# evandez/neuron-descriptions

Hardware: AMD Instinct MI355X
Metric: neuron-descriptions/sec (whole node), 4096 neurons x k=15 exemplars (higher is better)
Workload: dtype f32-equivalent: operands split into (hi,lo) f16 pairs (22 significant bits), 3 f16 MFMAs per product, f32 accumulate

## Files before the change

### neuron-descriptions_amd/csrc/chain.hip

```cpp
#include "common.h"

#include <cstdlib>

namespace milan {

typedef float f32x16 __attribute__((ext_vector_type(16)));
typedef float f32x4 __attribute__((ext_vector_type(4)));
typedef _Float16 f16x8 __attribute__((ext_vector_type(8)));

#define GLOBAL_AS __attribute__((address_space(1)))
#define LDS_AS __attribute__((address_space(3)))

namespace {

__device__ inline f16x8 h8(f32x4 v) { return __builtin_bit_cast(f16x8, v); }

__device__ inline void chain_split8(const float* v, f32x4* hi_out, f32x4* lo_out) {
  split8_rne(v, hi_out, lo_out);
}
__device__ inline void chain_join8(f32x4 hi, f32x4 lo, float* v) { join8_exact(hi, lo, v); }

constexpr int kSRow = 68;
constexpr int kTileFloats = 64 * 64;
constexpr int kConvMaxW = 56;
constexpr int kConvSlots = (256 + 2 * (kConvMaxW + 1) + 3) / 4 * 4;

template <int N>
__device__ __forceinline__ void wait_vmcnt() {
  asm volatile("s_waitcnt vmcnt(%0)" ::"n"(N) : "memory");
}

}

template <int P, int NW, bool RES_LDS, int KD, bool XACC, bool PROF = false, int NR = P,
          bool CONV = false, bool C1 = false>
__global__ __launch_bounds__(NW * 64, NW / 4) void chain_kernel(ChainArgs g) {
  long long tprof[8] = {0, 0, 0, 0, 0, 0, 0, 0};
  long long tlast = 0;
  auto stamp = [&](int k) {
    if constexpr (PROF) {
      const long long t = __builtin_readcyclecounter();
      tprof[k] += t - tlast;
      tlast = t;
    }
  };
  if constexpr (PROF) tlast = __builtin_readcyclecounter();
  constexpr int N3 = 4 * P, N1 = NR;
  constexpr int K3 = P + KD;
  constexpr int KS3 = K3 / 16;
  constexpr int NSLAB = N3 / 64;
  constexpr int T3 = K3 / 64;
  constexpr bool RES = KD == 0;
  static_assert(!(RES_LDS && !RES) && K3 % 64 == 0, "chain: configuration");
  constexpr int T1 = N1 / 64;
  constexpr int L = T3 + T1;
  constexpr int NT1 = N1 / 32;
  constexpr int STAGES = RES_LDS ? 7 : 4, AHEAD = STAGES - 1;
  constexpr int INFL = AHEAD - 2;
  constexpr int PIECES = 16 / NW;
  constexpr int C_OPS = RES_LDS ? 8 : (RES ? 10 : 2);
  static_assert(P % 64 == 0 && (NW == 4 || NW == 8), "chain: configuration");
  static_assert(!CONV || (P == 64 && NW == 8 && !RES_LDS), "chain: the conv front needs planes 64");
  static_assert(!C1 || CONV, "chain: c1 in front needs the conv front");
  constexpr int Q1 = C1 ? 1 : 0;
  constexpr int QC = CONV ? 9 + Q1 : 0;
  extern __shared__ __attribute__((aligned(16))) float smem[];

  const int tid = threadIdx.x;
  const int lane = tid & 63;
  const int wave = __builtin_amdgcn_readfirstlane(tid >> 6);
  const int px = lane & 31, half = lane >> 5;
  float sat = 0.f;
  float* ring = smem;
  float* strip = smem + STAGES * kTileFloats + wave * (32 * kSRow);
  float* rstrip = strip;
  float* biasl = smem + STAGES * kTileFloats + NW * (32 * kSRow);

  g.M = live_rows(g.m_live, g.m_live_mul, g.M);
  if ((long)blockIdx.x * (NW * 32) >= g.M) return;
  const long m0 = (long)blockIdx.x * (NW * 32) + wave * 32;
  const long mfrag = (m0 + px < g.M) ? m0 + px : (long)g.M - 1;
  const bool tail = (long)(blockIdx.x + 1) * (NW * 32) > g.M;

  const int lrow = lane >> 4;
  const int lpos = lane & 15;
  auto issue_tile = [&](int q) {
    constexpr int NTILES = QC + NSLAB * L;
    q = q < NTILES ? q : NTILES - 1;
    const float* base;
    long ld;
    if (C1 && q == 0) {
      base = g.W0; ld = 64;
    } else if (CONV && q < QC) {
      base = g.W2 + 64 * (q - Q1); ld = 9 * 64;
    } else {
      const int qc = q - QC;
      const int j = qc / L, qq = qc - j * L;
      if (qq < T3) { base = g.W3 + (long)(64 * j) * K3 + 64 * qq; ld = K3; }
      else { base = g.W1 + (long)(64 * (qq - T3)) * N3 + 64 * j; ld = N3; }
    }
    float* slot = ring + (q % STAGES) * kTileFloats;
#pragma unroll
    for (int i = 0; i < PIECES; ++i) {
      const int pc = wave * PIECES + i;
      const int rr = 4 * pc + lrow;
      const int c = lpos ^ (rr & 15);
      __builtin_amdgcn_global_load_lds(
          (const GLOBAL_AS void*)(base + (long)rr * ld + c * 4),
          (LDS_AS void*)(slot + pc * 256), 16, 0, 0);
    }
  };

  f32x4 t2h[KS3], t2l[KS3];
  float* const cin = smem + STAGES * kTileFloats;
  float* const czero = cin + kConvSlots * 64;
  f32x4 bias2v[CONV ? 8 : 1], bias0v[C1 ? 8 : 1];
  if constexpr (C1) {
#pragma unroll
    for (int s4 = 0; s4 < 4; ++s4) {
      bias0v[2 * s4] = *reinterpret_cast<const f32x4*>(g.bias0 + 16 * s4 + 8 * half);
      bias0v[2 * s4 + 1] = *reinterpret_cast<const f32x4*>(g.bias0 + 16 * s4 + 8 * half + 4);
    }
  }
  if constexpr (CONV) {
    const long wg0 = (long)blockIdx.x * (NW * 32);
    const int nslots = NW * 32 + 2 * (g.cw + 1);
    const int npieces = (nslots + 3) >> 2;
    for (int pc = wave; pc < npieces; pc += NW) {
      const int sl = 4 * pc + lrow;
      long m = wg0 - (g.cw + 1) + sl;
      m = m < 0 ? 0 : (m < g.M ? m : (long)g.M - 1);
      const int c = lpos ^ (sl & 15);
      __builtin_amdgcn_global_load_lds((const GLOBAL_AS void*)(g.C2in + m * 64 + c * 4),
                                       (LDS_AS void*)(cin + pc * 256), 16, 0, 0);
    }
    if (tid < 16) *reinterpret_cast<f32x4*>(czero + tid * 4) = f32x4{0.f, 0.f, 0.f, 0.f};
#pragma unroll
    for (int s4 = 0; s4 < 4; ++s4) {
      bias2v[2 * s4] = *reinterpret_cast<const f32x4*>(g.bias2 + 16 * s4 + 8 * half);
      bias2v[2 * s4 + 1] = *reinterpret_cast<const f32x4*>(g.bias2 + 16 * s4 + 8 * half + 4);
    }
  }
  {
    if constexpr (!CONV) {
    const float* tp = g.T2 + mfrag * P + half * 8;
#pragma unroll
    for (int s = 0; s < P / 16; ++s) {
      t2h[s] = *reinterpret_cast<const f32x4*>(tp + s * 16);
      t2l[s] = *reinterpret_cast<const f32x4*>(tp + s * 16 + 4);
    }
    }
    if constexpr (KD > 0) {
      const float* ap = g.A2 + mfrag * KD + half * 8;
#pragma unroll
      for (int s = 0; s < KD / 16; ++s) {
        t2h[P / 16 + s] = *reinterpret_cast<const f32x4*>(ap + s * 16);
        t2l[P / 16 + s] = *reinterpret_cast<const f32x4*>(ap + s * 16 + 4);
      }
    }
  }
  const int erow = lane >> 3, ecol = (lane & 7) * 8;
  f32x4 res[RES_LDS ? 1 : 4][2], bias3v[2];
  auto load_res = [&](int j) {
    if constexpr (!RES_LDS) {
      const int n = 64 * j + ecol;
      bias3v[0] = *reinterpret_cast<const f32x4*>(g.bias3 + n);
      bias3v[1] = *reinterpret_cast<const f32x4*>(g.bias3 + n + 4);
      if constexpr (!RES) return;
#pragma unroll
      for (int it = 0; it < 4; ++it) {
        long m = m0 + it * 8 + erow;
        m = m < g.M ? m : (long)g.M - 1;
        const float* rp = g.R + m * N3 + n;
        res[it][0] = *reinterpret_cast<const f32x4*>(rp);
        res[it][1] = *reinterpret_cast<const f32x4*>(rp + 4);
      }
      return;
    }
#pragma unroll
    for (int i = 0; i < 8; ++i) {
      const int r = 4 * i + lrow;
      long m = m0 + r;
      m = m < g.M ? m : (long)g.M - 1;
      const int c = lpos ^ (r & 1);
      __builtin_amdgcn_global_load_lds(
          (const GLOBAL_AS void*)(g.R + m * N3 + 64 * j + c * 4),
          (LDS_AS void*)(rstrip + i * 256), 16, 0, 0);
    }
  };
  if constexpr (RES_LDS) {
    for (int i = tid; i < N3; i += NW * 64) biasl[i] = g.bias3[i];
  }
  load_res(0);
#pragma unroll
  for (int t = 0; t < AHEAD; ++t) issue_tile(t);

  f32x16 acc1[NT1], acc1x[XACC ? NT1 : 1];
#pragma unroll
  for (int u = 0; u < NT1; ++u)
#pragma unroll
    for (int r = 0; r < 16; ++r) {
      acc1[u][r] = 0.f;
      if constexpr (XACC) acc1x[u][r] = 0.f;
    }

  const int fsw = px & 15;
  auto wfrag = [&](const float* slot, int t, int c) -> f32x4 {
    return *reinterpret_cast<const f32x4*>(slot + (32 * t + px) * 64 + ((c ^ fsw) << 2));
  };

  auto to_strip = [&](const f32x16& a, int t) {
#pragma unroll
    for (int qd = 0; qd < 4; ++qd) {
      f32x4 v = {a[4 * qd], a[4 * qd + 1], a[4 * qd + 2], a[4 * qd + 3]};
      *reinterpret_cast<f32x4*>(strip + px * kSRow + 32 * t + 8 * qd + 4 * half) = v;
    }
  };

  wait_vmcnt<INFL * PIECES>();
  asm volatile("s_waitcnt lgkmcnt(0)" ::: "memory");
  __builtin_amdgcn_s_barrier();
  stamp(0);
#pragma unroll
  for (int s = CONV ? P / 16 : 0; s < KS3; ++s)
    asm volatile("" : "+v"(t2h[s]), "+v"(t2l[s]));
  if constexpr (CONV) {
#pragma unroll
    for (int s = 0; s < 8; ++s) asm volatile("" : "+v"(bias2v[s]));
  }
  if constexpr (C1) {
#pragma unroll
    for (int s = 0; s < 8; ++s) asm volatile("" : "+v"(bias0v[s]));
  }

  f32x4 wh[2][2], wl[2][2];
  auto load_w = [&](const float* slot, int s, int buf) {
#pragma unroll
    for (int t = 0; t < 2; ++t) {
      if constexpr (NW == 4) {
        const float* ph = slot + (32 * t + px) * 64 + (((4 * s + 2 * half) ^ fsw) << 2);
        const float* pl = slot + (32 * t + px) * 64 + (((4 * s + 2 * half + 1) ^ fsw) << 2);
        asm volatile("ds_read_b128 %0, %1" : "=v"(wh[buf][t]) : "v"((LDS_AS const float*)ph) : "memory");
        asm volatile("ds_read_b128 %0, %1" : "=v"(wl[buf][t]) : "v"((LDS_AS const float*)pl) : "memory");
      } else {
        wh[buf][t] = wfrag(slot, t, 4 * s + 2 * half);
        wl[buf][t] = wfrag(slot, t, 4 * s + 2 * half + 1);
      }
    }
  };
  auto wait_w = [&](int buf) {
    if constexpr (NW == 4)
      asm volatile("s_waitcnt lgkmcnt(4)"
                   : "+v"(wh[buf][0]), "+v"(wh[buf][1]), "+v"(wl[buf][0]), "+v"(wl[buf][1])
                   :: "memory");
  };
  load_w(ring, 0, 0);

  if constexpr (CONV) {
    const int hw = g.ch * g.cw;
    const int img = (int)(mfrag / hw);
    const int rem = (int)(mfrag - (long)img * hw);
    const int y = rem / g.cw, x = rem - y * g.cw;
    const int slot0 = (int)(mfrag - (long)blockIdx.x * (NW * 32)) + g.cw + 1;
    LDS_AS const char* const cin_b = (LDS_AS const char*)cin;
    LDS_AS const char* const czero_b = (LDS_AS const char*)czero;
    f32x16 acc2[2];
#pragma unroll
    for (int t = 0; t < 2; ++t)
#pragma unroll
      for (int r = 0; r < 16; ++r) acc2[t][r] = 0.f;
    f32x4 bxh[2], bxl[2];
    LDS_AS const char* tbase = czero_b;
    unsigned tkey = 0;
    auto set_tap = [&](int tap) {
      const int kh = tap / 3, kw = tap - 3 * kh;
      const int yy = y + kh - 1, xx = x + kw - 1;
      const bool ok = (unsigned)yy < (unsigned)g.ch && (unsigned)xx < (unsigned)g.cw;
      const int sl = slot0 + (kh - 1) * g.cw + (kw - 1);
      tkey = (unsigned)(sl & 15) << 4;
      tbase = ok ? cin_b + sl * 256 : czero_b;
    };
    auto load_b = [&](int s, int buf) {
      const unsigned ch = (unsigned)((4 * s) << 4) + ((unsigned)(2 * half) << 4);
      bxh[buf] = *reinterpret_cast<LDS_AS const f32x4*>(tbase + (ch ^ tkey));
      bxl[buf] = *reinterpret_cast<LDS_AS const f32x4*>(tbase + ((ch + 16u) ^ tkey));
    };
    if constexpr (C1) {
      issue_tile(AHEAD);
      const int nslots = NW * 32 + 2 * (g.cw + 1);
      const int nblk = (nslots + 31) >> 5;
      const float* w0 = ring;
      for (int blk = wave; blk < nblk; blk += NW) {
        int sl = 32 * blk + px;
        const bool own = sl < nslots;
        sl = own ? sl : nslots - 1;
        LDS_AS char* const pb = (LDS_AS char*)cin + sl * 256;
        const unsigned key = (unsigned)(sl & 15) << 4;
        f32x4 xh[4], xl[4];
#pragma unroll
        for (int s = 0; s < 4; ++s) {
          const unsigned ch = (unsigned)((4 * s + 2 * half) << 4);
          xh[s] = *reinterpret_cast<LDS_AS const f32x4*>(pb + (ch ^ key));
          xl[s] = *reinterpret_cast<LDS_AS const f32x4*>(pb + ((ch + 16u) ^ key));
        }
#pragma unroll
        for (int t = 0; t < 2; ++t) {
          f32x16 a0, a0x;
#pragma unroll
          for (int r = 0; r < 16; ++r) { a0[r] = 0.f; a0x[r] = 0.f; }
#pragma unroll
          for (int s = 0; s < 4; ++s) {
            const f32x4 ah = wfrag(w0, t, 4 * s + 2 * half);
            const f32x4 al = wfrag(w0, t, 4 * s + 2 * half + 1);
            a0 = __builtin_amdgcn_mfma_f32_32x32x16_f16(h8(ah), h8(xh[s]), a0, 0, 0, 0);
            a0x = __builtin_amdgcn_mfma_f32_32x32x16_f16(h8(al), h8(xh[s]), a0x, 0, 0, 0);
            a0x = __builtin_amdgcn_mfma_f32_32x32x16_f16(h8(ah), h8(xl[s]), a0x, 0, 0, 0);
          }
          a0 = a0 + a0x;
#pragma unroll
          for (int sg = 0; sg < 2; ++sg) {
            float v[8];
#pragma unroll
            for (int i = 0; i < 4; ++i) {
              auto r = __builtin_amdgcn_permlane32_swap(__float_as_uint(a0[8 * sg + i]),
                                                        __float_as_uint(a0[8 * sg + 4 + i]),
                                                        false, false);
              v[i] = __uint_as_float(r[0]);
              v[4 + i] = __uint_as_float(r[1]);
            }
            const int s4 = 2 * t + sg;
#pragma unroll
            for (int e = 0; e < 4; ++e) {
              v[e] = __fmul_rn(v[e], g.scale0) + bias0v[2 * s4][e];
              v[4 + e] = __fmul_rn(v[4 + e], g.scale0) + bias0v[2 * s4 + 1][e];
            }
            f32x4 hi, lo;
            split8_relu_rne(v, &hi, &lo, &sat);
            const unsigned ch = (unsigned)((4 * s4 + 2 * half) << 4);
            if (own) {
              *reinterpret_cast<LDS_AS f32x4*>(pb + (ch ^ key)) = hi;
              *reinterpret_cast<LDS_AS f32x4*>(pb + ((ch + 16u) ^ key)) = lo;
            }
          }
        }
      }
      if (tail) wait_vmcnt<0>();
      else wait_vmcnt<INFL * PIECES>();
      asm volatile("s_waitcnt lgkmcnt(0)" ::: "memory");
      __builtin_amdgcn_s_barrier();
      load_w(ring + (Q1 % STAGES) * kTileFloats, 0, 0);
    }
    set_tap(0);
    load_b(0, 0);
#pragma unroll
    for (int q = Q1; q < QC; ++q) {
      issue_tile(q + AHEAD);
      const float* slot = ring + (q % STAGES) * kTileFloats;
      const float* next_slot = ring + ((q + 1) % STAGES) * kTileFloats;
#pragma unroll
      for (int s = 0; s < 4; ++s) {
        if (s < 3) {
          load_w(slot, s + 1, (s + 1) & 1);
          load_b(s + 1, (s + 1) & 1);
        } else {
          load_w(next_slot, 0, 0);
          if (q + 1 < QC) { set_tap(q + 1 - Q1); load_b(0, 0); }
        }
        const int b = s & 1;
        wait_w(b);
        acc2[0] = __builtin_amdgcn_mfma_f32_32x32x16_f16(h8(wl[b][0]), h8(bxh[b]), acc2[0], 0, 0, 0);
        acc2[1] = __builtin_amdgcn_mfma_f32_32x32x16_f16(h8(wl[b][1]), h8(bxh[b]), acc2[1], 0, 0, 0);
        acc2[0] = __builtin_amdgcn_mfma_f32_32x32x16_f16(h8(wh[b][0]), h8(bxl[b]), acc2[0], 0, 0, 0);
        acc2[1] = __builtin_amdgcn_mfma_f32_32x32x16_f16(h8(wh[b][1]), h8(bxl[b]), acc2[1], 0, 0, 0);
        acc2[0] = __builtin_amdgcn_mfma_f32_32x32x16_f16(h8(wh[b][0]), h8(bxh[b]), acc2[0], 0, 0, 0);
        acc2[1] = __builtin_amdgcn_mfma_f32_32x32x16_f16(h8(wh[b][1]), h8(bxh[b]), acc2[1], 0, 0, 0);
      }
      if (tail) wait_vmcnt<0>();
      else wait_vmcnt<INFL * PIECES>();
      __builtin_amdgcn_s_barrier();
    }
#pragma unroll
    for (int t = 0; t < 2; ++t)
#pragma unroll
      for (int sg = 0; sg < 2; ++sg) {
        float v[8];
#pragma unroll
        for (int i = 0; i < 4; ++i) {
          auto r = __builtin_amdgcn_permlane32_swap(__float_as_uint(acc2[t][8 * sg + i]),
                                                    __float_as_uint(acc2[t][8 * sg + 4 + i]),
                                                    false, false);
          v[i] = __uint_as_float(r[0]);
          v[4 + i] = __uint_as_float(r[1]);
        }
        const int s4 = 2 * t + sg;
#pragma unroll
        for (int e = 0; e < 4; ++e) {
          v[e] = __fmul_rn(v[e], g.scale2) + bias2v[2 * s4][e];
          v[4 + e] = __fmul_rn(v[4 + e], g.scale2) + bias2v[2 * s4 + 1][e];
        }
        split8_relu_rne(v, &t2h[s4], &t2l[s4], &sat);
      }
    stamp(7);
  }

  for (int j = 0; j < NSLAB; ++j) {
    f32x16 acc3[2];
#pragma unroll
    for (int t = 0; t < 2; ++t)
#pragma unroll
      for (int r = 0; r < 16; ++r) acc3[t][r] = 0.f;
    f32x4 xh[4], xl[4];
#pragma unroll
    for (int qq = 0; qq < L; ++qq) {
      const int q = QC + j * L + qq;
      issue_tile(q + AHEAD);
      stamp(1);
      const float* slot = ring + (q % STAGES) * kTileFloats;
      const float* next_slot = ring + ((q + 1) % STAGES) * kTileFloats;
#pragma unroll
      for (int s = 0; s < 4; ++s) {
        if (s < 3) load_w(slot, s + 1, (s + 1) & 1);
        else load_w(next_slot, 0, 0);
        const int b = s & 1;
        wait_w(b);
        if (qq < T3) {
          const int ks = 4 * qq + s;
          acc3[0] = __builtin_amdgcn_mfma_f32_32x32x16_f16(h8(wl[b][0]), h8(t2h[ks]), acc3[0], 0, 0, 0);
          acc3[1] = __builtin_amdgcn_mfma_f32_32x32x16_f16(h8(wl[b][1]), h8(t2h[ks]), acc3[1], 0, 0, 0);
          acc3[0] = __builtin_amdgcn_mfma_f32_32x32x16_f16(h8(wh[b][0]), h8(t2l[ks]), acc3[0], 0, 0, 0);
          acc3[1] = __builtin_amdgcn_mfma_f32_32x32x16_f16(h8(wh[b][1]), h8(t2l[ks]), acc3[1], 0, 0, 0);
          acc3[0] = __builtin_amdgcn_mfma_f32_32x32x16_f16(h8(wh[b][0]), h8(t2h[ks]), acc3[0], 0, 0, 0);
          acc3[1] = __builtin_amdgcn_mfma_f32_32x32x16_f16(h8(wh[b][1]), h8(t2h[ks]), acc3[1], 0, 0, 0);
        } else {
          const int u0 = 2 * (qq - T3);
          if constexpr (XACC) {
            acc1[u0] = __builtin_amdgcn_mfma_f32_32x32x16_f16(h8(wh[b][0]), h8(xh[s]), acc1[u0], 0, 0, 0);
            acc1[u0 + 1] = __builtin_amdgcn_mfma_f32_32x32x16_f16(h8(wh[b][1]), h8(xh[s]), acc1[u0 + 1], 0, 0, 0);
            acc1x[u0] = __builtin_amdgcn_mfma_f32_32x32x16_f16(h8(wl[b][0]), h8(xh[s]), acc1x[u0], 0, 0, 0);
            acc1x[u0 + 1] = __builtin_amdgcn_mfma_f32_32x32x16_f16(h8(wl[b][1]), h8(xh[s]), acc1x[u0 + 1], 0, 0, 0);
            acc1x[u0] = __builtin_amdgcn_mfma_f32_32x32x16_f16(h8(wh[b][0]), h8(xl[s]), acc1x[u0], 0, 0, 0);
            acc1x[u0 + 1] = __builtin_amdgcn_mfma_f32_32x32x16_f16(h8(wh[b][1]), h8(xl[s]), acc1x[u0 + 1], 0, 0, 0);
          } else {
            acc1[u0] = __builtin_amdgcn_mfma_f32_32x32x16_f16(h8(wl[b][0]), h8(xh[s]), acc1[u0], 0, 0, 0);
            acc1[u0 + 1] = __builtin_amdgcn_mfma_f32_32x32x16_f16(h8(wl[b][1]), h8(xh[s]), acc1[u0 + 1], 0, 0, 0);
            acc1[u0] = __builtin_amdgcn_mfma_f32_32x32x16_f16(h8(wh[b][0]), h8(xl[s]), acc1[u0], 0, 0, 0);
            acc1[u0 + 1] = __builtin_amdgcn_mfma_f32_32x32x16_f16(h8(wh[b][1]), h8(xl[s]), acc1[u0 + 1], 0, 0, 0);
            acc1[u0] = __builtin_amdgcn_mfma_f32_32x32x16_f16(h8(wh[b][0]), h8(xh[s]), acc1[u0], 0, 0, 0);
            acc1[u0 + 1] = __builtin_amdgcn_mfma_f32_32x32x16_f16(h8(wh[b][1]), h8(xh[s]), acc1[u0 + 1], 0, 0, 0);
          }
        }

      }
      stamp(2);
      if (qq == T3 - 1) {
        const int n = 64 * j + ecol;
        f32x4 bias0, bias1, rh4[4], rl4[4];
        if constexpr (RES_LDS) {
          wait_vmcnt<(L * PIECES < 63 ? L * PIECES : 63)>();
          bias0 = *reinterpret_cast<const f32x4*>(biasl + n);
          bias1 = *reinterpret_cast<const f32x4*>(biasl + n + 4);
#pragma unroll
          for (int it = 0; it < 4; ++it) {
            const int row = it * 8 + erow;
            const float* rp = rstrip + row * 64;
            const int rsw = row & 1;
            rh4[it] = *reinterpret_cast<const f32x4*>(rp + (((ecol >> 2)) ^ rsw) * 4);
            rl4[it] = *reinterpret_cast<const f32x4*>(rp + (((ecol >> 2) + 1) ^ rsw) * 4);
          }
        } else {
          bias0 = bias3v[0]; bias1 = bias3v[1];
        }
#pragma unroll
        for (int t = 0; t < 2; ++t) {
          acc3[t] = acc3[t] * g.scale3;
          to_strip(acc3[t], t);
        }
#pragma unroll
        for (int it = 0; it < 4; ++it) {
          const int row = it * 8 + erow;
          const long m = m0 + row;
          float* sp = strip + row * kSRow + ecol;
          const f32x4 v0 = *reinterpret_cast<const f32x4*>(sp);
          const f32x4 v1 = *reinterpret_cast<const f32x4*>(sp + 4);
          f32x4 rh, rl;
          if constexpr (RES_LDS) {
            rh = rh4[it]; rl = rl4[it];
          } else if constexpr (RES) {
            rh = res[it][0]; rl = res[it][1];
          }
          float v[8], a[8];
#pragma unroll
          for (int e = 0; e < 4; ++e) {
            v[e] = v0[e] + bias0[e];
            v[4 + e] = v1[e] + bias1[e];
          }
          if constexpr (RES) {
            chain_join8(rh, rl, a);
#pragma unroll
            for (int e = 0; e < 8; ++e) v[e] = v[e] + a[e];
          }
          f32x4 hi, lo;
          split8_relu_rne(v, &hi, &lo, &sat);
          if (m < g.M) {
            float* xp = g.X + m * N3 + n;
            *reinterpret_cast<f32x4*>(xp) = hi;
            *reinterpret_cast<f32x4*>(xp + 4) = lo;
          }
          *reinterpret_cast<f32x4*>(sp) = hi;
          *reinterpret_cast<f32x4*>(sp + 4) = lo;
        }
        if constexpr (!RES_LDS) load_res(j + 1 < NSLAB ? j + 1 : j);
#pragma unroll
        for (int s = 0; s < 4; ++s) {
          const float* fp = strip + px * kSRow + (2 * s + half) * 8;
          xh[s] = *reinterpret_cast<const f32x4*>(fp);
          xl[s] = *reinterpret_cast<const f32x4*>(fp + 4);
        }
        if constexpr (RES_LDS) {
          asm volatile("s_waitcnt lgkmcnt(0)"
                       : "+v"(xh[0]), "+v"(xh[1]), "+v"(xh[2]), "+v"(xh[3]),
                         "+v"(xl[0]), "+v"(xl[1]), "+v"(xl[2]), "+v"(xl[3])
                       :: "memory");
          load_res(j + 1 < NSLAB ? j + 1 : j);
        }
      }
      stamp(3);
      {
        constexpr auto has_c = [](int i) { return ((i % L) + L) % L == T3 - 1; };
        int c_later = 0, c_first = 0;
#pragma unroll
        for (int d = 0; d <= INFL; ++d) {
          c_later += has_c(qq - d) ? 1 : 0;
          c_first += (qq - d >= 0 && has_c(qq - d)) ? 1 : 0;
        }
        const int cnt = (j == 0) ? c_first : c_later;
        constexpr int B = INFL * PIECES;
        if (tail) {
          wait_vmcnt<0>();
        } else {
          switch (cnt) {
            case 0: wait_vmcnt<B>(); break;
            case 1: wait_vmcnt<(B + C_OPS < 63 ? B + C_OPS : 63)>(); break;
            case 2: wait_vmcnt<(B + 2 * C_OPS < 63 ? B + 2 * C_OPS : 63)>(); break;
            default: wait_vmcnt<(B + 3 * C_OPS < 63 ? B + 3 * C_OPS : 63)>(); break;
          }
        }
      }
      stamp(4);
      __builtin_amdgcn_s_barrier();
      stamp(5);
    }
  }
  wait_vmcnt<0>();
  __builtin_amdgcn_s_barrier();

#pragma unroll
  for (int cidx = 0; cidx < NT1 / 2; ++cidx) {
#pragma unroll
    for (int t = 0; t < 2; ++t) {
      if constexpr (XACC) acc1[2 * cidx + t] = acc1[2 * cidx + t] + acc1x[2 * cidx + t];
      acc1[2 * cidx + t] = acc1[2 * cidx + t] * g.scale1;
      to_strip(acc1[2 * cidx + t], t);
    }
    const int n = 64 * cidx + ecol;
    const f32x4 b0 = *reinterpret_cast<const f32x4*>(g.bias1 + n);
    const f32x4 b1 = *reinterpret_cast<const f32x4*>(g.bias1 + n + 4);
#pragma unroll
    for (int it = 0; it < 4; ++it) {
      const int row = it * 8 + erow;
      const long m = m0 + row;
      const float* sp = strip + row * kSRow + ecol;
      const f32x4 v0 = *reinterpret_cast<const f32x4*>(sp);
      const f32x4 v1 = *reinterpret_cast<const f32x4*>(sp + 4);
      float v[8];
#pragma unroll
      for (int e = 0; e < 4; ++e) {
        v[e] = v0[e] + b0[e];
        v[4 + e] = v1[e] + b1[e];
      }
      f32x4 hi, lo;
      split8_relu_rne(v, &hi, &lo, &sat);
      if (m < g.M) {
        float* tp = g.T1 + m * N1 + n;
        *reinterpret_cast<f32x4*>(tp) = hi;
        *reinterpret_cast<f32x4*>(tp + 4) = lo;
      }
    }
  }
  report_saturation(g.status, sat);
  if constexpr (PROF) {
    stamp(6);
    if (tid == 0 && g.prof)
      for (int k = 0; k < 8; ++k) g.prof[(long)blockIdx.x * 8 + k] = tprof[k];
  }
}


bool chain_conv_supported(int P, int KD, int NR, int h, int w) {
  return P == 64 && chain_supported(P, KD, NR) && h >= 1 && w >= 1 && w <= kConvMaxW;
}

bool chain_conv_c1_supported(int P, int KD, int NR, int h, int w) {
  return chain_conv_supported(P, KD, NR, h, w) && KD == 64 && NR == 64;
}

bool chain_supported(int P, int KD, int NR) {
  if (NR == 2 * P) return KD == 0 && P == 64;
  if (NR != P) return false;
  if (KD == 0) return P == 64 || P == 128 || P == 256;
  return P == 64 && KD == 64;
}

template <int P, int NW, bool RES_LDS, int KD, bool XACC, bool PROF = false, int NR = P,
          bool CONV = false, bool C1 = false>
static int launch_chain_cfg(const ChainArgs& a, hipStream_t s) {
  size_t lds = sizeof(float) * (size_t)((RES_LDS ? 7 : 4) * kTileFloats +
                                        NW * 32 * kSRow + (RES_LDS ? 4 * P : 0));
  if (CONV) {
    const size_t with_region = sizeof(float) * (size_t)(4 * kTileFloats + kConvSlots * 64 + 64);
    lds = lds > with_region ? lds : with_region;
  }
  auto kern = chain_kernel<P, NW, RES_LDS, KD, XACC, PROF, NR, CONV, C1>;
  MILAN_TRY(ensure_lds_attr(reinterpret_cast<const void*>(kern), (int)lds));
  const int rows = NW * 32;
  const int grid = (a.M + rows - 1) / rows;
  hipLaunchKernelGGL(kern, dim3(grid), dim3(NW * 64), lds, s, a);
  MILAN_CHECK_HIP(hipGetLastError());
  return 0;
}

int launch_chain3(const ChainArgs& a, hipStream_t s);

int launch_chain(const ChainArgs& a0, hipStream_t s) {
  ChainArgs a = a0;
  if (a.status == nullptr) a.status = status_word();
  const int NR = a.NR ? a.NR : a.P;
  MILAN_REQUIRE(chain_supported(a.P, a.KD, NR) && a.M > 0, MILAN_ERR_SHAPE,
                "chain: unsupported planes %d (+%d) -> %d", a.P, a.KD, NR);
  auto al = [](const void* p) { return (reinterpret_cast<uintptr_t>(p) & 15) == 0; };
  const bool conv = a.C2in != nullptr;
  MILAN_REQUIRE(!conv || (chain_conv_supported(a.P, a.KD, NR, a.ch, a.cw) && a.W2 && a.bias2 &&
                          al(a.C2in) && al(a.W2) && al(a.bias2) && a.C2in != a.T1 &&
                          a.M % (a.ch * a.cw) == 0),
                MILAN_ERR_SHAPE, "chain: unsupported 3x3 front (%d x %d images)", a.ch, a.cw);
  const bool c1 = conv && a.W0 != nullptr;
  MILAN_REQUIRE(!c1 || (chain_conv_c1_supported(a.P, a.KD, NR, a.ch, a.cw) && a.bias0 && al(a.W0) &&
                        al(a.bias0)),
                MILAN_ERR_SHAPE, "chain: unsupported c1 front");
  MILAN_REQUIRE((conv || al(a.T2)) && al(a.W3) && al(a.bias3) && al(a.X) && al(a.W1) &&
                    al(a.bias1) && al(a.T1) &&
                    (a.KD ? (a.A2 && al(a.A2) && !a.R) : (a.R && al(a.R))),
                MILAN_ERR_SHAPE, "chain: operands must be 16-byte aligned");
  const double M = a.M, P = a.P, K3 = a.P + a.KD, R1 = NR;
  void* rec = gemm_profile_begin(
      2.0 * M * (4 * P) * (K3 + R1) + (conv ? 2.0 * M * 64 * 576 : 0.0) + (c1 ? 2.0 * M * 64 * 64 : 0.0),
      4.0 * (M * K3 + M * 4 * P * (a.KD ? 1 : 2) + M * R1 + 4 * P * (K3 + R1) +
             (conv ? 64.0 * 576 : 0.0)), s);
  profile_tag_kernel(a.P == 256 ? MILAN_KERNEL_CHAIN_WIDE
                                : (conv ? MILAN_KERNEL_BNECK : MILAN_KERNEL_CHAIN));
  int r;
#if MILAN_EXPERIMENTS
  if (conv && a.KD == 0 && NR == 64 && a.prof)
    r = launch_chain_cfg<64, 8, false, 0, true, true, 64, true>(a, s);
  else
#endif
  if (conv && NR == 128) r = launch_chain_cfg<64, 8, false, 0, false, false, 128, true>(a, s);
  else if (conv && a.KD == 0) r = launch_chain_cfg<64, 8, false, 0, true, false, 64, true>(a, s);
  else if (c1) r = launch_chain_cfg<64, 8, false, 64, true, false, 64, true, true>(a, s);
  else if (conv) r = launch_chain_cfg<64, 8, false, 64, true, false, 64, true>(a, s);
  else if (a.P == 256) r = launch_chain3(a, s);
  else if (a.P == 128) r = launch_chain_cfg<128, 8, false, 0, false>(a, s);
  else if (NR == 128) r = launch_chain_cfg<64, 8, false, 0, false, false, 128>(a, s);
  else if (a.KD == 0) r = launch_chain_cfg<64, 8, false, 0, true>(a, s);
  else r = launch_chain_cfg<64, 8, false, 64, true>(a, s);
  gemm_profile_end(rec, s);
  return r;
}

}
```

Baseline: 1440.

## Make chain kernel persistent with XCD-aware tile walk and cross-tile prefetch

Result: no change. 1453 (median of 6 runs) (+0.9%).

```diff
diff --git a/neuron-descriptions_amd/csrc/chain.hip b/neuron-descriptions_amd/csrc/chain.hip
--- a/neuron-descriptions_amd/csrc/chain.hip
+++ b/neuron-descriptions_amd/csrc/chain.hip
@@ -34,8 +34,8 @@
 
 template <int P, int NW, bool RES_LDS, int KD, bool XACC, bool PROF = false, int NR = P,
           bool CONV = false, bool C1 = false>
-__global__ __launch_bounds__(NW * 64, NW / 4) void chain_kernel(ChainArgs g) {
-  long long tprof[8] = {0, 0, 0, 0, 0, 0, 0, 0};
+__global__ __launch_bounds__(NW * 64, NW / 4) void chain_kernel(ChainArgs g, int walk) {
+  long long tprof[10] = {0, 0, 0, 0, 0, 0, 0, 0, 0, 0};
   long long tlast = 0;
   auto stamp = [&](int k) {
     if constexpr (PROF) {
@@ -69,7 +69,7 @@
   const int tid = threadIdx.x;
   const int lane = tid & 63;
   const int wave = __builtin_amdgcn_readfirstlane(tid >> 6);
-  const int px = lane & 31, half = lane >> 5;
+  int px = lane & 31, half = lane >> 5;
   float sat = 0.f;
   float* ring = smem;
   float* strip = smem + STAGES * kTileFloats + wave * (32 * kSRow);
@@ -77,16 +77,42 @@
   float* biasl = smem + STAGES * kTileFloats + NW * (32 * kSRow);
 
   g.M = live_rows(g.m_live, g.m_live_mul, g.M);
-  if ((long)blockIdx.x * (NW * 32) >= g.M) return;
-  const long m0 = (long)blockIdx.x * (NW * 32) + wave * 32;
-  const long mfrag = (m0 + px < g.M) ? m0 + px : (long)g.M - 1;
-  const bool tail = (long)(blockIdx.x + 1) * (NW * 32) > g.M;
-
-  const int lrow = lane >> 4;
-  const int lpos = lane & 15;
+  const int ntile = (g.M + NW * 32 - 1) / (NW * 32);
+  int tile = blockIdx.x, tstep = 1, tend = ntile < tile + 1 ? ntile : tile + 1;
+  if (walk) {
+    const int G = gridDim.x, nxcd = G < 8 ? G : 8;
+    const int xcd = tile % nxcd;
+    tstep = (G - xcd + nxcd - 1) / nxcd;
+    tend = (int)((long)ntile * (xcd + 1) / nxcd);
+    tile = (int)((long)ntile * xcd / nxcd) + (int)blockIdx.x / nxcd;
+  }
+  if (tile >= tend) return;
+  long m0, mfrag;
+  bool tail;
+  auto set_tile = [&](int t) {
+    m0 = (long)t * (NW * 32) + wave * 32;
+    mfrag = (m0 + px < g.M) ? m0 + px : (long)g.M - 1;
+    tail = (long)(t + 1) * (NW * 32) > g.M;
+  };
+  set_tile(tile);
+  int qb = 0;
+  bool more;
+  int tilen;
+  long m0n;
+  auto set_next = [&]() {
+    more = tile + tstep < tend;
+    tilen = more ? tile + tstep : tile;
+    m0n = (long)tilen * (NW * 32) + wave * 32;
+  };
+  set_next();
+
+  int lrow = lane >> 4;
+  int lpos = lane & 15;
+  constexpr int NTILES = QC + NSLAB * L;
+  auto ring_slot = [&](int q) { return ring + ((q + qb) % STAGES) * kTileFloats; };
   auto issue_tile = [&](int q) {
-    constexpr int NTILES = QC + NSLAB * L;
-    q = q < NTILES ? q : NTILES - 1;
+    float* slot = ring_slot(q);
+    if (q >= NTILES) q = more ? q - NTILES : NTILES - 1;
     const float* base;
     long ld;
     if (C1 && q == 0) {
@@ -99,7 +125,6 @@
       if (qq < T3) { base = g.W3 + (long)(64 * j) * K3 + 64 * qq; ld = K3; }
       else { base = g.W1 + (long)(64 * (qq - T3)) * N3 + 64 * j; ld = N3; }
     }
-    float* slot = ring + (q % STAGES) * kTileFloats;
 #pragma unroll
     for (int i = 0; i < PIECES; ++i) {
       const int pc = wave * PIECES + i;
@@ -115,53 +140,72 @@
   float* const cin = smem + STAGES * kTileFloats;
   float* const czero = cin + kConvSlots * 64;
   f32x4 bias2v[CONV ? 8 : 1], bias0v[C1 ? 8 : 1];
-  if constexpr (C1) {
-#pragma unroll
-    for (int s4 = 0; s4 < 4; ++s4) {
-      bias0v[2 * s4] = *reinterpret_cast<const f32x4*>(g.bias0 + 16 * s4 + 8 * half);
-      bias0v[2 * s4 + 1] = *reinterpret_cast<const f32x4*>(g.bias0 + 16 * s4 + 8 * half + 4);
-    }
-  }
+  auto load_front_bias = [&]() {
+    if constexpr (C1) {
+#pragma unroll
+      for (int s4 = 0; s4 < 4; ++s4) {
+        bias0v[2 * s4] = *reinterpret_cast<const f32x4*>(g.bias0 + 16 * s4 + 8 * half);
+        bias0v[2 * s4 + 1] = *reinterpret_cast<const f32x4*>(g.bias0 + 16 * s4 + 8 * half + 4);
+      }
+    }
+    if constexpr (CONV) {
+#pragma unroll
+      for (int s4 = 0; s4 < 4; ++s4) {
+        bias2v[2 * s4] = *reinterpret_cast<const f32x4*>(g.bias2 + 16 * s4 + 8 * half);
+        bias2v[2 * s4 + 1] = *reinterpret_cast<const f32x4*>(g.bias2 + 16 * s4 + 8 * half + 4);
+      }
+    }
+  };
+  constexpr int kStripPieces = NW * 32 * kSRow / 256;
+  constexpr int kMaxPieces = kConvSlots / 4;
+  constexpr int kEarlyRounds = (kMaxPieces - kStripPieces + NW - 1) / NW;
+  static_assert(!CONV || NW * 32 * kSRow % 256 == 0, "chain: strips end on a piece boundary");
+  const int npieces = CONV ? (NW * 32 + 2 * (g.cw + 1) + 3) >> 2 : 0;
+  auto region_piece = [&](int t, int pc) {
+    const int sl = 4 * pc + lrow;
+    long m = (long)t * (NW * 32) - (g.cw + 1) + sl;
+    m = m < 0 ? 0 : (m < g.M ? m : (long)g.M - 1);
+    const int c = lpos ^ (sl & 15);
+    __builtin_amdgcn_global_load_lds((const GLOBAL_AS void*)(g.C2in + m * 64 + c * 4),
+                                     (LDS_AS void*)(cin + pc * 256), 16, 0, 0);
+  };
+  auto issue_region = [&](int t, int pc_end) {
+    for (int pc = wave; pc < pc_end; pc += NW) region_piece(t, pc);
+  };
+  auto issue_region_early = [&](int t) {
+#pragma unroll
+    for (int i = 0; i < kEarlyRounds; ++i) {
+      const int pc = kStripPieces + i * NW + wave;
+      region_piece(t, pc < npieces ? pc : kMaxPieces - 1);
+    }
+  };
   if constexpr (CONV) {
-    const long wg0 = (long)blockIdx.x * (NW * 32);
-    const int nslots = NW * 32 + 2 * (g.cw + 1);
-    const int npieces = (nslots + 3) >> 2;
-    for (int pc = wave; pc < npieces; pc += NW) {
-      const int sl = 4 * pc + lrow;
-      long m = wg0 - (g.cw + 1) + sl;
-      m = m < 0 ? 0 : (m < g.M ? m : (long)g.M - 1);
-      const int c = lpos ^ (sl & 15);
-      __builtin_amdgcn_global_load_lds((const GLOBAL_AS void*)(g.C2in + m * 64 + c * 4),
-                                       (LDS_AS void*)(cin + pc * 256), 16, 0, 0);
-    }
+    issue_region(tile, npieces);
     if (tid < 16) *reinterpret_cast<f32x4*>(czero + tid * 4) = f32x4{0.f, 0.f, 0.f, 0.f};
-#pragma unroll
-    for (int s4 = 0; s4 < 4; ++s4) {
-      bias2v[2 * s4] = *reinterpret_cast<const f32x4*>(g.bias2 + 16 * s4 + 8 * half);
-      bias2v[2 * s4 + 1] = *reinterpret_cast<const f32x4*>(g.bias2 + 16 * s4 + 8 * half + 4);
-    }
-  }
-  {
+    load_front_bias();
+  }
+  auto load_t2 = [&](long mf) {
     if constexpr (!CONV) {
-    const float* tp = g.T2 + mfrag * P + half * 8;
-#pragma unroll
-    for (int s = 0; s < P / 16; ++s) {
-      t2h[s] = *reinterpret_cast<const f32x4*>(tp + s * 16);
-      t2l[s] = *reinterpret_cast<const f32x4*>(tp + s * 16 + 4);
-    }
+      const float* tp = g.T2 + mf * P + half * 8;
+#pragma unroll
+      for (int s = 0; s < P / 16; ++s) {
+        t2h[s] = *reinterpret_cast<const f32x4*>(tp + s * 16);
+        t2l[s] = *reinterpret_cast<const f32x4*>(tp + s * 16 + 4);
+      }
     }
     if constexpr (KD > 0) {
-      const float* ap = g.A2 + mfrag * KD + half * 8;
+      const float* ap = g.A2 + mf * KD + half * 8;
 #pragma unroll
       for (int s = 0; s < KD / 16; ++s) {
         t2h[P / 16 + s] = *reinterpret_cast<const f32x4*>(ap + s * 16);
         t2l[P / 16 + s] = *reinterpret_cast<const f32x4*>(ap + s * 16 + 4);
       }
     }
-  }
-  const int erow = lane >> 3, ecol = (lane & 7) * 8;
+  };
+  load_t2(mfrag);
+  int erow = lane >> 3, ecol = (lane & 7) * 8;
   f32x4 res[RES_LDS ? 1 : 4][2], bias3v[2];
-  auto load_res = [&](int j) {
+  auto load_res = [&](int j, long mw) {
     if constexpr (!RES_LDS) {
       const int n = 64 * j + ecol;
       bias3v[0] = *reinterpret_cast<const f32x4*>(g.bias3 + n);
@@ -169,7 +213,7 @@
       if constexpr (!RES) return;
 #pragma unroll
       for (int it = 0; it < 4; ++it) {
-        long m = m0 + it * 8 + erow;
+        long m = mw + it * 8 + erow;
         m = m < g.M ? m : (long)g.M - 1;
         const float* rp = g.R + m * N3 + n;
         res[it][0] = *reinterpret_cast<const f32x4*>(rp);
@@ -180,7 +224,7 @@
 #pragma unroll
     for (int i = 0; i < 8; ++i) {
       const int r = 4 * i + lrow;
-      long m = m0 + r;
+      long m = mw + r;
       m = m < g.M ? m : (long)g.M - 1;
       const int c = lpos ^ (r & 1);
       __builtin_amdgcn_global_load_lds(
@@ -191,11 +235,46 @@
   if constexpr (RES_LDS) {
     for (int i = tid; i < N3; i += NW * 64) biasl[i] = g.bias3[i];
   }
-  load_res(0);
+  load_res(0, m0);
 #pragma unroll
   for (int t = 0; t < AHEAD; ++t) issue_tile(t);
 
   f32x16 acc1[NT1], acc1x[XACC ? NT1 : 1];
+
+  int fsw = px & 15;
+  auto wfrag = [&](const float* slot, int t, int c) -> f32x4 {
+    return *reinterpret_cast<const f32x4*>(slot + (32 * t + px) * 64 + ((c ^ fsw) << 2));
+  };
+
+  auto to_strip = [&](const f32x16& a, int t) {
+#pragma unroll
+    for (int qd = 0; qd < 4; ++qd) {
+      f32x4 v = {a[4 * qd], a[4 * qd + 1], a[4 * qd + 2], a[4 * qd + 3]};
+      *reinterpret_cast<f32x4*>(strip + px * kSRow + 32 * t + 8 * qd + 4 * half) = v;
+    }
+  };
+
+  wait_vmcnt<INFL * PIECES>();
+
+  f32x4 wh[2][2], wl[2][2];
+
+  auto roles = [&]() {
+    int l = lane;
+    asm volatile("" : "+v"(l));
+    px = l & 31; half = l >> 5;
+    lrow = l >> 4; lpos = l & 15;
+    erow = l >> 3; ecol = (l & 7) * 8;
+    fsw = px & 15;
+  };
+  for (int ntl = 0;; ++ntl) {
+  roles();
+  asm volatile("s_waitcnt lgkmcnt(0)" ::: "memory");
+  __builtin_amdgcn_s_barrier();
+  if constexpr (PROF) {
+    if (ntl == 0) stamp(0);
+    else stamp(8);
+    tprof[9] += 1;
+  }
 #pragma unroll
   for (int u = 0; u < NT1; ++u)
 #pragma unroll
@@ -203,24 +282,6 @@
       acc1[u][r] = 0.f;
       if constexpr (XACC) acc1x[u][r] = 0.f;
     }
-
-  const int fsw = px & 15;
-  auto wfrag = [&](const float* slot, int t, int c) -> f32x4 {
-    return *reinterpret_cast<const f32x4*>(slot + (32 * t + px) * 64 + ((c ^ fsw) << 2));
-  };
-
-  auto to_strip = [&](const f32x16& a, int t) {
-#pragma unroll
-    for (int qd = 0; qd < 4; ++qd) {
-      f32x4 v = {a[4 * qd], a[4 * qd + 1], a[4 * qd + 2], a[4 * qd + 3]};
-      *reinterpret_cast<f32x4*>(strip + px * kSRow + 32 * t + 8 * qd + 4 * half) = v;
-    }
-  };
-
-  wait_vmcnt<INFL * PIECES>();
-  asm volatile("s_waitcnt lgkmcnt(0)" ::: "memory");
-  __builtin_amdgcn_s_barrier();
-  stamp(0);
 #pragma unroll
   for (int s = CONV ? P / 16 : 0; s < KS3; ++s)
     asm volatile("" : "+v"(t2h[s]), "+v"(t2l[s]));
@@ -233,7 +294,6 @@
     for (int s = 0; s < 8; ++s) asm volatile("" : "+v"(bias0v[s]));
   }
 
-  f32x4 wh[2][2], wl[2][2];
   auto load_w = [&](const float* slot, int s, int buf) {
 #pragma unroll
     for (int t = 0; t < 2; ++t) {
@@ -254,14 +314,14 @@
                    : "+v"(wh[buf][0]), "+v"(wh[buf][1]), "+v"(wl[buf][0]), "+v"(wl[buf][1])
                    :: "memory");
   };
-  load_w(ring, 0, 0);
+  load_w(ring_slot(0), 0, 0);
 
   if constexpr (CONV) {
     const int hw = g.ch * g.cw;
     const int img = (int)(mfrag / hw);
     const int rem = (int)(mfrag - (long)img * hw);
     const int y = rem / g.cw, x = rem - y * g.cw;
-    const int slot0 = (int)(mfrag - (long)blockIdx.x * (NW * 32)) + g.cw + 1;
+    const int slot0 = (int)(mfrag - (long)tile * (NW * 32)) + g.cw + 1;
     LDS_AS const char* const cin_b = (LDS_AS const char*)cin;
     LDS_AS const char* const czero_b = (LDS_AS const char*)czero;
     f32x16 acc2[2];
@@ -286,10 +346,11 @@
       bxl[buf] = *reinterpret_cast<LDS_AS const f32x4*>(tbase + ((ch + 16u) ^ tkey));
     };
     if constexpr (C1) {
+      roles();
       issue_tile(AHEAD);
       const int nslots = NW * 32 + 2 * (g.cw + 1);
       const int nblk = (nslots + 31) >> 5;
-      const float* w0 = ring;
+      const float* w0 = ring_slot(0);
       for (int blk = wave; blk < nblk; blk += NW) {
         int sl = 32 * blk + px;
         const bool own = sl < nslots;
@@ -348,15 +409,16 @@
       else wait_vmcnt<INFL * PIECES>();
       asm volatile("s_waitcnt lgkmcnt(0)" ::: "memory");
       __builtin_amdgcn_s_barrier();
-      load_w(ring + (Q1 % STAGES) * kTileFloats, 0, 0);
-    }
+      load_w(ring_slot(Q1), 0, 0);
+    }
+    roles();
     set_tap(0);
     load_b(0, 0);
 #pragma unroll
     for (int q = Q1; q < QC; ++q) {
       issue_tile(q + AHEAD);
-      const float* slot = ring + (q % STAGES) * kTileFloats;
-      const float* next_slot = ring + ((q + 1) % STAGES) * kTileFloats;
+      const float* slot = ring_slot(q);
+      const float* next_slot = ring_slot(q + 1);
 #pragma unroll
       for (int s = 0; s < 4; ++s) {
         if (s < 3) {
@@ -403,6 +465,7 @@
     stamp(7);
   }
 
+  roles();
   for (int j = 0; j < NSLAB; ++j) {
     f32x16 acc3[2];
 #pragma unroll
@@ -414,9 +477,12 @@
     for (int qq = 0; qq < L; ++qq) {
       const int q = QC + j * L + qq;
       issue_tile(q + AHEAD);
+      if constexpr (CONV) {
+        if (qq == 0 && j == NSLAB - 1 && more) issue_region_early(tilen);
+      }
       stamp(1);
-      const float* slot = ring + (q % STAGES) * kTileFloats;
-      const float* next_slot = ring + ((q + 1) % STAGES) * kTileFloats;
+      const float* slot = ring_slot(q);
+      const float* next_slot = ring_slot(q + 1);
 #pragma unroll
       for (int s = 0; s < 4; ++s) {
         if (s < 3) load_w(slot, s + 1, (s + 1) & 1);
@@ -509,7 +575,7 @@
           *reinterpret_cast<f32x4*>(sp) = hi;
           *reinterpret_cast<f32x4*>(sp + 4) = lo;
         }
-        if constexpr (!RES_LDS) load_res(j + 1 < NSLAB ? j + 1 : j);
+        if constexpr (!RES_LDS) load_res(j + 1 < NSLAB ? j + 1 : 0, j + 1 < NSLAB ? m0 : m0n);
 #pragma unroll
         for (int s = 0; s < 4; ++s) {
           const float* fp = strip + px * kSRow + (2 * s + half) * 8;
@@ -521,7 +587,7 @@
                        : "+v"(xh[0]), "+v"(xh[1]), "+v"(xh[2]), "+v"(xh[3]),
                          "+v"(xl[0]), "+v"(xl[1]), "+v"(xl[2]), "+v"(xl[3])
                        :: "memory");
-          load_res(j + 1 < NSLAB ? j + 1 : j);
+          load_res(j + 1 < NSLAB ? j + 1 : 0, j + 1 < NSLAB ? m0 : m0n);
         }
       }
       stamp(3);
@@ -534,9 +600,17 @@
           c_first += (qq - d >= 0 && has_c(qq - d)) ? 1 : 0;
         }
         const int cnt = (j == 0) ? c_first : c_later;
-        constexpr int B = INFL * PIECES;
+        const bool early = CONV && qq <= INFL && j == NSLAB - 1 && more;
+        constexpr int B = INFL * PIECES, BE = B + (CONV ? kEarlyRounds : 0);
         if (tail) {
           wait_vmcnt<0>();
+        } else if (early) {
+          switch (cnt) {
+            case 0: wait_vmcnt<BE>(); break;
+            case 1: wait_vmcnt<(BE + C_OPS < 63 ? BE + C_OPS : 63)>(); break;
+            case 2: wait_vmcnt<(BE + 2 * C_OPS < 63 ? BE + 2 * C_OPS : 63)>(); break;
+            default: wait_vmcnt<(BE + 3 * C_OPS < 63 ? BE + 3 * C_OPS : 63)>(); break;
+          }
         } else {
           switch (cnt) {
             case 0: wait_vmcnt<B>(); break;
@@ -554,6 +628,16 @@
   wait_vmcnt<0>();
   __builtin_amdgcn_s_barrier();
 
+  roles();
+  f32x4 b1v[NT1 / 2][2];
+#pragma unroll
+  for (int cidx = 0; cidx < NT1 / 2; ++cidx) {
+    b1v[cidx][0] = *reinterpret_cast<const f32x4*>(g.bias1 + 64 * cidx + ecol);
+    b1v[cidx][1] = *reinterpret_cast<const f32x4*>(g.bias1 + 64 * cidx + ecol + 4);
+  }
+  if constexpr (!CONV || KD > 0) {
+    if (more) load_t2(m0n + px < g.M ? m0n + px : (long)g.M - 1);
+  }
 #pragma unroll
   for (int cidx = 0; cidx < NT1 / 2; ++cidx) {
 #pragma unroll
@@ -563,8 +647,7 @@
       to_strip(acc1[2 * cidx + t], t);
     }
     const int n = 64 * cidx + ecol;
-    const f32x4 b0 = *reinterpret_cast<const f32x4*>(g.bias1 + n);
-    const f32x4 b1 = *reinterpret_cast<const f32x4*>(g.bias1 + n + 4);
+    const f32x4 b0 = b1v[cidx][0], b1 = b1v[cidx][1];
 #pragma unroll
     for (int it = 0; it < 4; ++it) {
       const int row = it * 8 + erow;
@@ -587,11 +670,24 @@
       }
     }
   }
+  stamp(6);
+  if (!more) break;
+  roles();
+  tile = tilen;
+  set_tile(tile);
+  set_next();
+  qb = (qb + NTILES) % STAGES;
+  if constexpr (CONV) {
+    __builtin_amdgcn_s_barrier();
+    load_front_bias();
+    issue_region(tile, npieces < kStripPieces ? npieces : kStripPieces);
+    wait_vmcnt<0>();
+  }
+  }
   report_saturation(g.status, sat);
   if constexpr (PROF) {
-    stamp(6);
     if (tid == 0 && g.prof)
-      for (int k = 0; k < 8; ++k) g.prof[(long)blockIdx.x * 8 + k] = tprof[k];
+      for (int k = 0; k < 10; ++k) g.prof[(long)blockIdx.x * 16 + k] = tprof[k];
   }
 }
 
@@ -623,8 +719,18 @@
   auto kern = chain_kernel<P, NW, RES_LDS, KD, XACC, PROF, NR, CONV, C1>;
   MILAN_TRY(ensure_lds_attr(reinterpret_cast<const void*>(kern), (int)lds));
   const int rows = NW * 32;
-  const int grid = (a.M + rows - 1) / rows;
-  hipLaunchKernelGGL(kern, dim3(grid), dim3(NW * 64), lds, s, a);
+  int grid = (a.M + rows - 1) / rows;
+  const char* e = getenv("MILAN_CHAIN_PERSIST");
+  const int walk = !RES_LDS && (e ? atoi(e) : 1) ? 1 : 0;
+  if (walk) {
+    int cus = 0;
+    MILAN_TRY(device_cus8(&cus));
+    const char* w = getenv("MILAN_CHAIN_PERSIST_WGS");
+    const int cap = w ? atoi(w) : 0;
+    if (cap > 0 && cap < cus) cus = cap;
+    if (grid > cus) grid = cus;
+  }
+  hipLaunchKernelGGL(kern, dim3(grid), dim3(NW * 64), lds, s, a, walk);
   MILAN_CHECK_HIP(hipGetLastError());
   return 0;
 }
```
